# YuePanEdward/GH-ICP

Measured on AMD Instinct MI355X. Metric: registered_pairs_per_sec, higher is better.
Workload: dtype f64

## Files before the change

gh-icp_amd/csrc/bsc.hip:

```cpp
#include "frontend.h"
#include "devmath.h"
#include "bsc_dev.h"

namespace {

__global__ __launch_bounds__(BT) void k_bsc(GridArgs G, const int* __restrict__ kp, BscConst C, uint8_t* __restrict__ feat, float* __restrict__ lcs) {
  gh_bsc_keypoint(G, C, (int)blockIdx.x, C.K, feat, lcs);
}

__global__ __launch_bounds__(256) void k_bsc_origins(const float* __restrict__ xyz, int stride, const int* __restrict__ kp, int K, float* __restrict__ lcs) {
  const int k = blockIdx.x * 256 + threadIdx.x;
  if (k >= K) return;
  const long long s = kp[k];
  lcs[(size_t)k * 12 + 9] = xyz[s * stride];
  lcs[(size_t)k * 12 + 10] = xyz[s * stride + 1];
  lcs[(size_t)k * 12 + 11] = xyz[s * stride + 2];
}

}

int gh_bsc_make_const(ghicp_ctx* ctx, float R, int dof, const int32_t* pattern_host, BscConst* out, float* r_search) {
  BscConst C;
  memset(&C, 0, sizeof(C));
  C.R = R;
  const double rs = std::sqrt(3.0) * (double)R;
  C.r2s = (float)(rs * rs);
  C.u = 2 * R / 7;
  const float delta = (float)(C.u * 0.5);
  C.den = 2 * delta * delta;
  C.r2c = (float)((1.5 * (double)C.u) * (1.5 * (double)C.u));
  C.area = (float)(M_PI * (double)R * (double)R);
  C.radius_w = std::sqrt(2.0) * (double)R;
  int ex = 0;
  (void)std::frexp((double)R * 0.5, &ex);
  C.dunit = std::ldexp(1.0, 24 - ex);
  C.dinv = std::ldexp(1.0, ex - 54);
  for (int i = 0; i < 7; i++) C.centre[i] = (float)((i + 0.5) * (double)C.u - (double)R);
  for (int i = 0; i < 98; i++) {
    C.pattern[i] = pattern_host[i];
    if (C.pattern[i] < 0 || C.pattern[i] > 48) return ctx->fail(GHICP_ERR_ARG, "BSC sample pattern entry %d out of [0,48]", i);
  }
  C.K = 0;
  C.nvar = (dof > 4) ? 4 : (dof > 0 ? 2 : 1);
  *out = C;
  *r_search = (float)rs;
  return GHICP_OK;
}

int gh_bsc_dev(ghicp_ctx* ctx, const float* xyz, long long m, int stride, const int32_t* kp, long long K, float R, int dof, const int32_t* pattern_host,
               uint8_t* feat, float* lcs) {
  if (K <= 0) return GHICP_OK;
  hipStream_t s = ctx->stream;
  BscConst C;
  float r_search_f = 0.f;
  GH_TRY(gh_bsc_make_const(ctx, R, dof, pattern_host, &C, &r_search_f));
  C.K = (int)K;
  DeviceGrid G;
  const GridSlots sl = {B_GRID2_KEYS, B_GRID2_KEYS2, B_GRID2_VALS, B_GRID2_VALS2, B_GRID2_START, B_GRID2_PTS};
  GH_TRY(gh_grid_build(ctx, xyz, m, stride, r_search_f * 1.0001f, sl, &G));
  GH_HIP(hipMemsetAsync(feat, 0, (size_t)4 * K * 56, s));
  hipLaunchKernelGGL(k_bsc_origins, dim3(cdiv(K, 256)), dim3(256), 0, s, xyz, stride, kp, (int)K, lcs);
  GridArgs A = {G.d, G.pts, G.start};
  hipEvent_t kt = ctx->kt_begin(KT_BSC);
  hipLaunchKernelGGL(k_bsc, dim3((unsigned)K), dim3(BT), 0, s, A, kp, C, feat, lcs);
  ctx->kt_end(KT_BSC, kt);
  GH_HIP(hipGetLastError());
  return GHICP_OK;
}

extern "C" int ghicp_bsc_encode(ghicp_ctx* ctx, const float* xyz, int64_t m, int stride, const int32_t* kp_idx, int64_t k, float radius, int dof,
                                const int32_t* pattern, uint8_t* feat, float* lcs) {
  GH_ENTER(ctx);
  GH_ARG(m >= 0 && m < (1ll << 31) - 2 && k >= 0 && k <= m && stride >= 3 && radius > 0.f && pattern != nullptr);
  Stager sg(ctx);
  const float* d;
  const int32_t* dk;
  uint8_t* df;
  float* dl;
  GH_TRY(sg.in_cloud(xyz, (size_t)m * stride, &d));
  GH_TRY(sg.in(kp_idx, (size_t)k, &dk));
  GH_TRY(sg.out(feat, (size_t)4 * k * 56, &df));
  GH_TRY(sg.out(lcs, (size_t)k * 12, &dl));
  GH_TRY(gh_bsc_dev(ctx, d, m, stride, dk, k, radius, dof, pattern, df, dl));
  return sg.finish();
}
```

gh-icp_amd/csrc/bsc_dev.h:

```cpp
#pragma once
#include "grid.h"
#include "devmath.h"
#include "bsc_exp_table.h"

struct BscConst {
  float R, r2s, u, den, r2c, area;
  double radius_w;
  double dunit, dinv;
  float centre[7];
  int pattern[98];
  int K, nvar;
};

constexpr int BT = 256;
constexpr int BSC_CAP = 2048;
constexpr int BSC_CHUNK = 512;

int gh_bsc_make_const(ghicp_ctx* ctx, float R, int dof, const int32_t* pattern_host, BscConst* out, float* r_search);

static __device__ const double gh_bsc_exp_tab[145] = {GH_BSC_EXP_TABLE};
__device__ inline float gh_bsc_expf(float xf, const double* __restrict__ tab) {
  const double x = (double)xf;
  int j = (int)(x * -32.0 + 0.5);
  j = j < 0 ? 0 : (j > 144 ? 144 : j);
  const double s = x + (double)j * 0.03125;
  double p = s * (1.0 / 720.0) + (1.0 / 120.0);
  p = s * p + (1.0 / 24.0);
  p = s * p + (1.0 / 6.0);
  p = s * p + 0.5;
  p = s * p + 1.0;
  p = s * p + 1.0;
  return (float)(tab[j] * p);
}

__device__ inline void gh_bsc_depth_add(unsigned long long* __restrict__ lo64, unsigned* __restrict__ carry, float depth, float ew, double dunit) {
  const unsigned d_off = (unsigned)((int)((double)depth * dunit) + (1 << 27));
  const unsigned w_int = (unsigned)((double)ew * 1073741824.0);
  const unsigned long long term = (unsigned long long)d_off * (unsigned long long)w_int;
  const unsigned long long old = atomicAdd(lo64, term);
  if (old + term < old) atomicAdd(carry, 1u);
}
__device__ inline double gh_bsc_depth_sum(unsigned long long lo64, unsigned carry, double pnum, double dinv) {
  const unsigned __int128 acc = ((unsigned __int128)carry << 64) | (unsigned __int128)lo64;
  const unsigned __int128 shift = (unsigned __int128)(unsigned long long)(pnum * 1073741824.0) << 27;
  const bool neg = acc < shift;
  const unsigned __int128 mag = neg ? shift - acc : acc - shift;
  const double d = (double)(unsigned long long)(mag >> 32) * 4294967296.0 + (double)(unsigned long long)(mag & 0xFFFFFFFFull);
  return (neg ? -d : d) * dinv;
}

__device__ inline int rearr_src(int type, int k) {
  switch (type) {
    case 1: return 48 - k;
    case 2: return (6 - k / 7) * 7 + k % 7;
    default: return (k / 7) * 7 + 6 - k % 7;
  }
}

__device__ inline void gh_bsc_keypoint(const GridArgs& G, const BscConst& C, int kk, int K, uint8_t* __restrict__ feat, float* __restrict__ lcs) {

  __shared__ double red[16];
  __shared__ double s_pnum[147], s_exp[145];
  __shared__ unsigned long long s_dlo[147];
  __shared__ unsigned s_dcarry[147];
  __shared__ float s_weight[147], s_depth[147];
  __shared__ float s_axes[9];
  __shared__ double s_stat[3][4];
  __shared__ unsigned s_bits[4][16];
  __shared__ float4 s_pts[BSC_CHUNK];
  __shared__ int s_scan[17];
  __shared__ float s_centre[8];
  const int tid = threadIdx.x;
  const float qx = lcs[(size_t)kk * 12 + 9], qy = lcs[(size_t)kk * 12 + 10], qz = lcs[(size_t)kk * 12 + 11];
  const int cx = gh_cell_coord(qx, G.d.mn[0], G.d.inv, G.d.dim[0]);
  const int cy = gh_cell_coord(qy, G.d.mn[1], G.d.inv, G.d.dim[1]);
  const int cz = gh_cell_coord(qz, G.d.mn[2], G.d.inv, G.d.dim[2]);

  double sx = 0, sy = 0, sz = 0, sw = 0;
  int cnt = 0;
  gh_for_runs(G.d, G.start, cx, cy, cz, [&](unsigned b, unsigned e) {
    for (unsigned q = b + tid; q < e; q += BT) {
      const float4 P = G.pts[q];
      const float dx = qx - P.x, dy = qy - P.y, dz = qz - P.z;
      float d2 = dx * dx;
      d2 += dy * dy;
      d2 += dz * dz;
      if (d2 < C.r2s) {
        cnt++;
        sx += (double)P.x; sy += (double)P.y; sz += (double)P.z;
        sw += C.radius_w - (double)sqrtf(d2);
      }
    }
  });
  sx = gh_block_sum(sx, red); sy = gh_block_sum(sy, red); sz = gh_block_sum(sz, red); sw = gh_block_sum(sw, red);
  int mm;
  const int my_base = gh_block_excl_scan(cnt, s_scan, &mm);
  const double mx = sx / (double)mm, my = sy / (double)mm, mz = sz / (double)mm;
  const bool packed = mm <= BSC_CAP;
  auto fill_chunk = [&](int c0) {
    int w = my_base;
    gh_for_runs(G.d, G.start, cx, cy, cz, [&](unsigned b, unsigned e) {
      for (unsigned q = b + tid; q < e; q += BT) {
        const float4 P = G.pts[q];
        const float dx = qx - P.x, dy = qy - P.y, dz = qz - P.z;
        float d2 = dx * dx;
        d2 += dy * dy;
        d2 += dz * dz;
        if (d2 < C.r2s) {
          if (w >= c0 && w < c0 + BSC_CHUNK) s_pts[w - c0] = make_float4(P.x, P.y, P.z, d2);
          w++;
        }
      }
    });
    __syncthreads();
  };

  double c00 = 0, c01 = 0, c02 = 0, c11 = 0, c12 = 0, c22 = 0;
  if (mm >= 3 && packed) {
    for (int c0 = 0; c0 < mm; c0 += BSC_CHUNK) {
      fill_chunk(c0);
      const int cn = min(BSC_CHUNK, mm - c0);
      for (int t = tid; t < cn; t += BT) {
        const float4 P = s_pts[t];
        const double w = (double)(float)(C.radius_w - (double)sqrtf(P.w));
        const double ex = (double)P.x - mx, ey = (double)P.y - my, ez = (double)P.z - mz;
        c00 += w * ex * ex; c01 += w * ex * ey; c02 += w * ex * ez;
        c11 += w * ey * ey; c12 += w * ey * ez; c22 += w * ez * ez;
      }
      __syncthreads();
    }
  } else if (mm >= 3) {
    gh_for_runs(G.d, G.start, cx, cy, cz, [&](unsigned b, unsigned e) {
      for (unsigned q = b + tid; q < e; q += BT) {
        const float4 P = G.pts[q];
        const float dx = qx - P.x, dy = qy - P.y, dz = qz - P.z;
        float d2 = dx * dx;
        d2 += dy * dy;
        d2 += dz * dz;
        if (d2 < C.r2s) {
          const double w = (double)(float)(C.radius_w - (double)sqrtf(d2));
          const double ex = (double)P.x - mx, ey = (double)P.y - my, ez = (double)P.z - mz;
          c00 += w * ex * ex; c01 += w * ex * ey; c02 += w * ex * ez;
          c11 += w * ey * ey; c12 += w * ey * ez; c22 += w * ez * ez;
        }
      }
    });
  }
  if (mm >= 3) {
    c00 = gh_block_sum(c00, red); c01 = gh_block_sum(c01, red); c02 = gh_block_sum(c02, red);
    c11 = gh_block_sum(c11, red); c12 = gh_block_sum(c12, red); c22 = gh_block_sum(c22, red);
  }
  if (tid == 0) {
    float X[3] = {1, 0, 0}, Y[3] = {0, 1, 0}, Z[3] = {0, 0, 1};
    if (mm >= 3) {
      const float da = (float)sw;
      double Cq[6] = {c00, c01, c02, c11, c12, c22};
      gh_quant_grid(Cq, 6);
      double a00 = (double)((float)Cq[0] / da), a01 = (double)((float)Cq[1] / da), a02 = (double)((float)Cq[2] / da),
             a11 = (double)((float)Cq[3] / da), a12 = (double)((float)Cq[4] / da), a22 = (double)((float)Cq[5] / da);
      double V[9];
      gh_jacobi3(a00, a01, a02, a11, a12, a22, V);
      const double ev[3] = {a00, a11, a22};
      int imax = 0, imin = 0;
      for (int i = 0; i < 3; i++) {
        if ((float)ev[i] > (float)ev[imax]) imax = i;
        if ((float)ev[i] < (float)ev[imin]) imin = i;
      }
      float P[3], N[3];
      for (int which = 0; which < 2; which++) {
        const int col = which == 0 ? imax : imin;
        const double e[3] = {V[0 * 3 + col], V[1 * 3 + col], V[2 * 3 + col]};
        int b = 0;
        if (fabs(e[1]) > fabs(e[b])) b = 1;
        if (fabs(e[2]) > fabs(e[b])) b = 2;
        const double sg = (e[b] < 0) ? -1.0 : 1.0;
        float* o = which == 0 ? P : N;
        for (int d = 0; d < 3; d++) o[d] = (float)(sg * e[d]);
      }
      const float M0 = P[1] * N[2] - P[2] * N[1], M1 = P[2] * N[0] - P[0] * N[2], M2 = P[0] * N[1] - P[1] * N[0];
      X[0] = P[0]; X[1] = P[1]; X[2] = P[2];
      Y[0] = M0; Y[1] = M1; Y[2] = M2;
      Z[0] = X[1] * Y[2] - X[2] * Y[1];
      Z[1] = X[2] * Y[0] - X[0] * Y[2];
      Z[2] = X[0] * Y[1] - X[1] * Y[0];
      const float nx = sqrtf((X[0] * X[0] + X[1] * X[1]) + X[2] * X[2]);
      const float ny = sqrtf((Y[0] * Y[0] + Y[1] * Y[1]) + Y[2] * Y[2]);
      for (int d = 0; d < 3; d++) { X[d] = X[d] / nx; Y[d] = Y[d] / ny; }
    }
    for (int d = 0; d < 3; d++) { s_axes[d] = X[d]; s_axes[3 + d] = Y[d]; s_axes[6 + d] = Z[d]; }
    float* o = &lcs[(size_t)kk * 12];
    for (int d = 0; d < 3; d++) { o[d] = X[d]; o[3 + d] = Y[d]; o[6 + d] = Z[d]; }
  }
  for (int i = tid; i < 147; i += BT) { s_pnum[i] = 0.0; s_dlo[i] = 0ull; s_dcarry[i] = 0u; }
  for (int i = tid; i < 145; i += BT) s_exp[i] = gh_bsc_exp_tab[i];
  if (tid < 7) s_centre[tid] = C.centre[tid];
  if (tid < 64) s_bits[tid >> 4][tid & 15] = 0u;
  __syncthreads();
  const float X0 = s_axes[0], X1 = s_axes[1], X2 = s_axes[2], Y0 = s_axes[3], Y1 = s_axes[4], Y2 = s_axes[5], Z0 = s_axes[6], Z1 = s_axes[7],
              Z2 = s_axes[8];

  auto splat = [&](float px, float py, float pz) {
    const float d0 = px - qx, d1 = py - qy, d2v = pz - qz;
    const float loc[3] = {(X0 * d0 + X1 * d1) + X2 * d2v, (Y0 * d0 + Y1 * d1) + Y2 * d2v, (Z0 * d0 + Z1 * d1) + Z2 * d2v};
#pragma unroll
    for (int pl = 0; pl < 3; pl++) {
      const float a = loc[pl == 2 ? 1 : 0], bb = loc[pl == 0 ? 1 : 2];
      const float depth = loc[pl == 0 ? 2 : (pl == 1 ? 1 : 0)] + C.R;
      for (int j = 0; j < 7; j++) {
        const float dy = bb - C.centre[j];
        const float dy2 = dy * dy;
        if (!(dy2 < C.r2c)) continue;
        for (int i = 0; i < 7; i++) {
          const float dx = a - C.centre[i];
          float dd = dx * dx;
          dd += dy2;
          if (dd < C.r2c) {
            const float ew = gh_bsc_expf(-dd / C.den, s_exp);
            atomicAdd(&s_pnum[i + 7 * j + 49 * pl], (double)ew);
            gh_bsc_depth_add(&s_dlo[i + 7 * j + 49 * pl], &s_dcarry[i + 7 * j + 49 * pl], depth, ew, C.dunit);
          }
        }
      }
    }
  };
  if (packed) {
    const int wave = tid >> 6, lane = tid & 63;
    const int sub = lane / 9, slot = lane % 9;
    const int di = slot % 3 - 1, dj = slot / 3 - 1;
    const float inv_u = 1.0f / C.u;
    for (int c0 = 0; c0 < mm; c0 += BSC_CHUNK) {
    fill_chunk(c0);
    const int cn = min(BSC_CHUNK, mm - c0);
    for (int t = tid; t < cn; t += BT) {
      const float4 P = s_pts[t];
      const float d0 = P.x - qx, d1 = P.y - qy, d2v = P.z - qz;
      s_pts[t] = make_float4((X0 * d0 + X1 * d1) + X2 * d2v, (Y0 * d0 + Y1 * d1) + Y2 * d2v, (Z0 * d0 + Z1 * d1) + Z2 * d2v, 0.f);
    }
    __syncthreads();
    const int nitem = cn * 3;
    for (int base = 0; base < nitem; base += 28) {
      const int w = base + wave * 7 + sub;
      if (lane < 63 && w < nitem) {
        const int t = w / 3, pl = w - 3 * t;
        const float4 L = s_pts[t];
        const float a = pl == 2 ? L.y : L.x, bb = pl == 0 ? L.y : L.z;
        const float depth = (pl == 0 ? L.z : (pl == 1 ? L.y : L.x)) + C.R;
        const float ta = (a + C.R) * inv_u, tb = (bb + C.R) * inv_u;
        const float fla = floorf(ta), flb = floorf(tb);
        const int bi = (int)fla, bj = (int)flb;
        auto cell = [&](int ci, int cj) {
          if (ci < 0 || ci >= 7 || cj < 0 || cj >= 7) return;
          const float dy = bb - s_centre[cj];
          const float dy2 = dy * dy;
          const float dx = a - s_centre[ci];
          float dd = dx * dx;
          dd += dy2;
          if (dy2 < C.r2c && dd < C.r2c) {
            const float ew = gh_bsc_expf(-dd / C.den, s_exp);
            atomicAdd(&s_pnum[ci + 7 * cj + 49 * pl], (double)ew);
            gh_bsc_depth_add(&s_dlo[ci + 7 * cj + 49 * pl], &s_dcarry[ci + 7 * cj + 49 * pl], depth, ew, C.dunit);
          }
        };
        cell(bi + di, bj + dj);
        const float fa = ta - fla, fb = tb - flb;
        if (fa < 1e-4f || fa > 0.9999f || fb < 1e-4f || fb > 0.9999f) {
          bool fx = false, fy = false;
          const int i2 = bi + 2 * di, j2 = bj + 2 * dj;
          if (di != 0 && i2 >= 0 && i2 < 7) { const float dx = a - s_centre[i2]; fx = dx * dx < C.r2c; }
          if (dj != 0 && j2 >= 0 && j2 < 7) { const float dy = bb - s_centre[j2]; fy = dy * dy < C.r2c; }
          if (fx) cell(i2, bj + dj);
          if (fy) cell(bi + di, j2);
          if (fx && fy) cell(i2, j2);
        }
      }
    }
    __syncthreads();
    }
  } else {
    gh_for_runs(G.d, G.start, cx, cy, cz, [&](unsigned b, unsigned e) {
      for (unsigned q = b + tid; q < e; q += BT) {
        const float4 P = G.pts[q];
        const float tx = qx - P.x, ty = qy - P.y, tz = qz - P.z;
        float d2 = tx * tx;
        d2 += ty * ty;
        d2 += tz * tz;
        if (!(d2 < C.r2s)) continue;
        splat(P.x, P.y, P.z);
      }
    });
  }
  __syncthreads();

  if (tid < 147) {
    const float ndens = (float)mm / C.area;
    float avg = (float)gh_bsc_depth_sum(s_dlo[tid], s_dcarry[tid], s_pnum[tid], C.dinv);
    avg = (s_pnum[tid] == 0.0) ? 0.0f : (float)((double)avg / s_pnum[tid]);
    const float garea = C.u * C.u;
    const float gdens = (float)(s_pnum[tid] / (double)garea);
    s_weight[tid] = (ndens != 0.0f) ? gdens / ndens : 0.0f;
    s_depth[tid] = avg;
  }
  __syncthreads();
  if (tid < 3) {
    const int off = 49 * tid;
    double avg_d = 0, var_d = 0, avg_w = 0, var_w = 0;
    for (int i = 0; i < 49; i++) {
      const int a = C.pattern[2 * i] + off, b = C.pattern[2 * i + 1] + off;
      avg_d += (double)(s_depth[a] - s_depth[b]);
      avg_w += (double)(s_weight[a] - s_weight[b]);
    }
    avg_d /= 49; avg_w /= 49;
    for (int i = 0; i < 49; i++) {
      const int a = C.pattern[2 * i] + off, b = C.pattern[2 * i + 1] + off;
      const double dd = (double)(s_depth[a] - s_depth[b]), dw = (double)(s_weight[a] - s_weight[b]);
      var_d += (dd - avg_d) * (dd - avg_d);
      var_w += (dw - avg_w) * (dw - avg_w);
    }
    var_d /= 49; var_w /= 49;
    s_stat[tid][0] = avg_d; s_stat[tid][1] = sqrt(var_d); s_stat[tid][2] = avg_w; s_stat[tid][3] = sqrt(var_w);
  }
  __syncthreads();
  for (int base = 0; base < 448; base += BT) {
    const int k = base + tid;
    for (int v = 0; v < C.nvar; v++) {
      bool bit = false;
      if (v == 0) {
        if (k < 147) bit = s_weight[k] > 0.1f;
        else if (k < 441) {
          const int r = k - 147, pl = r / 98, p = (r % 98) >> 1, off = 49 * pl;
          const int a = C.pattern[2 * p], b = C.pattern[2 * p + 1];
          if ((r & 1) == 0) {
            const double dd = (double)(s_depth[a + off] - s_depth[b + off]);
            bit = fabs(dd - s_stat[pl][0]) > s_stat[pl][1];
          } else if (!(s_weight[a] < 0.1f && s_weight[b] < 0.1f)) {
            const double dw = (double)(s_weight[a + off] - s_weight[b + off]);
            bit = fabs(dw - s_stat[pl][2]) > s_stat[pl][3];
          }
        }
      } else if (k >= 147 && k < 294) {
        static const int TR[4][3] = {{0, 0, 0}, {1, 2, 2}, {3, 2, 1}, {2, 1, 3}};
        const int r = k - 147, pl = r / 49, kk2 = r % 49;
        bit = s_weight[49 * pl + rearr_src(TR[v][pl], kk2)] > 0.1f;
      }
      const unsigned long long bal = __ballot(bit);
      if ((tid & 63) == 0 && k < 448) {
        s_bits[v][k >> 5] = (unsigned)bal;
        if (k + 32 < 448) s_bits[v][(k >> 5) + 1] = (unsigned)(bal >> 32);
      }
    }
  }
  __syncthreads();
  if (tid < 14 * C.nvar) {
    const int v = tid / 14, w = tid % 14;
    reinterpret_cast<unsigned*>(feat)[((size_t)v * K + kk) * 14 + w] = s_bits[v][w];
  }
}
```

Before: 441.9.

## Replace double weight atomics with integer sums and division with reciprocal refinement

Replaces the per-cell double-precision atomicAdd of Gaussian weights with a 64-bit integer weight sum built from the float's bit pattern, which also feeds the depth-offset computation. The division by den becomes a precomputed reciprocal with two FMA refinement steps, and the depth unit conversion moves from double to float. It also skips reloading the point chunk when all neighbours fit in one resident chunk. These changes aim to cut slow double atomics and double math in the hot splat loop, at the risk of small numeric differences in the weight and depth quantisation.

Result: no change. 444.6, median of 6 (+0.6%).

```diff
diff --git a/gh-icp_amd/csrc/bsc.hip b/gh-icp_amd/csrc/bsc.hip
--- a/gh-icp_amd/csrc/bsc.hip
+++ b/gh-icp_amd/csrc/bsc.hip
@@ -28,6 +28,7 @@
   C.u = 2 * R / 7;
   const float delta = (float)(C.u * 0.5);
   C.den = 2 * delta * delta;
+  gh_bsc_quot_const(C.den, &C.rden, &C.dd_min);
   C.r2c = (float)((1.5 * (double)C.u) * (1.5 * (double)C.u));
   C.area = (float)(M_PI * (double)R * (double)R);
   C.radius_w = std::sqrt(2.0) * (double)R;
diff --git a/gh-icp_amd/csrc/bsc_dev.h b/gh-icp_amd/csrc/bsc_dev.h
--- a/gh-icp_amd/csrc/bsc_dev.h
+++ b/gh-icp_amd/csrc/bsc_dev.h
@@ -2,9 +2,11 @@
 #include "grid.h"
 #include "devmath.h"
 #include "bsc_exp_table.h"
+#include "bsc_weight.h"
 
 struct BscConst {
   float R, r2s, u, den, r2c, area;
+  float rden, dd_min;
   double radius_w;
   double dunit, dinv;
   float centre[7];
@@ -33,16 +35,17 @@
   return (float)(tab[j] * p);
 }
 
-__device__ inline void gh_bsc_depth_add(unsigned long long* __restrict__ lo64, unsigned* __restrict__ carry, float depth, float ew, double dunit) {
-  const unsigned d_off = (unsigned)((int)((double)depth * dunit) + (1 << 27));
-  const unsigned w_int = (unsigned)((double)ew * 1073741824.0);
+__device__ inline unsigned gh_bsc_depth_units(float depth, float dunit) { return (unsigned)((int)(depth * dunit) + (1 << 27)); }
+__device__ inline void gh_bsc_cell_add(unsigned long long* __restrict__ wsum, unsigned long long* __restrict__ lo64, unsigned* __restrict__ carry, unsigned d_off, float ew) {
+  const unsigned w_int = gh_bsc_weight_int(ew);
+  atomicAdd(wsum, (unsigned long long)w_int);
   const unsigned long long term = (unsigned long long)d_off * (unsigned long long)w_int;
   const unsigned long long old = atomicAdd(lo64, term);
   if (old + term < old) atomicAdd(carry, 1u);
 }
-__device__ inline double gh_bsc_depth_sum(unsigned long long lo64, unsigned carry, double pnum, double dinv) {
+__device__ inline double gh_bsc_depth_sum(unsigned long long lo64, unsigned carry, unsigned long long wsum, double dinv) {
   const unsigned __int128 acc = ((unsigned __int128)carry << 64) | (unsigned __int128)lo64;
-  const unsigned __int128 shift = (unsigned __int128)(unsigned long long)(pnum * 1073741824.0) << 27;
+  const unsigned __int128 shift = (unsigned __int128)wsum << 27;
   const bool neg = acc < shift;
   const unsigned __int128 mag = neg ? shift - acc : acc - shift;
   const double d = (double)(unsigned long long)(mag >> 32) * 4294967296.0 + (double)(unsigned long long)(mag & 0xFFFFFFFFull);
@@ -60,8 +63,8 @@
 __device__ inline void gh_bsc_keypoint(const GridArgs& G, const BscConst& C, int kk, int K, uint8_t* __restrict__ feat, float* __restrict__ lcs) {
 
   __shared__ double red[16];
-  __shared__ double s_pnum[147], s_exp[145];
-  __shared__ unsigned long long s_dlo[147];
+  __shared__ double s_exp[145];
+  __shared__ unsigned long long s_wsum[147], s_dlo[147];
   __shared__ unsigned s_dcarry[147];
   __shared__ float s_weight[147], s_depth[147];
   __shared__ float s_axes[9];
@@ -191,11 +194,12 @@
     float* o = &lcs[(size_t)kk * 12];
     for (int d = 0; d < 3; d++) { o[d] = X[d]; o[3 + d] = Y[d]; o[6 + d] = Z[d]; }
   }
-  for (int i = tid; i < 147; i += BT) { s_pnum[i] = 0.0; s_dlo[i] = 0ull; s_dcarry[i] = 0u; }
+  for (int i = tid; i < 147; i += BT) { s_wsum[i] = 0ull; s_dlo[i] = 0ull; s_dcarry[i] = 0u; }
   for (int i = tid; i < 145; i += BT) s_exp[i] = gh_bsc_exp_tab[i];
   if (tid < 7) s_centre[tid] = C.centre[tid];
   if (tid < 64) s_bits[tid >> 4][tid & 15] = 0u;
   __syncthreads();
+  const float dunit = (float)C.dunit;
   const float X0 = s_axes[0], X1 = s_axes[1], X2 = s_axes[2], Y0 = s_axes[3], Y1 = s_axes[4], Y2 = s_axes[5], Z0 = s_axes[6], Z1 = s_axes[7],
               Z2 = s_axes[8];
 
@@ -205,7 +209,7 @@
 #pragma unroll
     for (int pl = 0; pl < 3; pl++) {
       const float a = loc[pl == 2 ? 1 : 0], bb = loc[pl == 0 ? 1 : 2];
-      const float depth = loc[pl == 0 ? 2 : (pl == 1 ? 1 : 0)] + C.R;
+      const unsigned d_off = gh_bsc_depth_units(loc[pl == 0 ? 2 : (pl == 1 ? 1 : 0)] + C.R, dunit);
       for (int j = 0; j < 7; j++) {
         const float dy = bb - C.centre[j];
         const float dy2 = dy * dy;
@@ -215,9 +219,8 @@
           float dd = dx * dx;
           dd += dy2;
           if (dd < C.r2c) {
-            const float ew = gh_bsc_expf(-dd / C.den, s_exp);
-            atomicAdd(&s_pnum[i + 7 * j + 49 * pl], (double)ew);
-            gh_bsc_depth_add(&s_dlo[i + 7 * j + 49 * pl], &s_dcarry[i + 7 * j + 49 * pl], depth, ew, C.dunit);
+            const float ew = gh_bsc_expf(gh_bsc_neg_quot(dd, C.den, C.rden, C.dd_min), s_exp);
+            gh_bsc_cell_add(&s_wsum[i + 7 * j + 49 * pl], &s_dlo[i + 7 * j + 49 * pl], &s_dcarry[i + 7 * j + 49 * pl], d_off, ew);
           }
         }
       }
@@ -228,8 +231,9 @@
     const int sub = lane / 9, slot = lane % 9;
     const int di = slot % 3 - 1, dj = slot / 3 - 1;
     const float inv_u = 1.0f / C.u;
+    const bool resident = mm >= 3 && mm <= BSC_CHUNK;
     for (int c0 = 0; c0 < mm; c0 += BSC_CHUNK) {
-    fill_chunk(c0);
+    if (!resident) fill_chunk(c0);
     const int cn = min(BSC_CHUNK, mm - c0);
     for (int t = tid; t < cn; t += BT) {
       const float4 P = s_pts[t];
@@ -244,7 +248,7 @@
         const int t = w / 3, pl = w - 3 * t;
         const float4 L = s_pts[t];
         const float a = pl == 2 ? L.y : L.x, bb = pl == 0 ? L.y : L.z;
-        const float depth = (pl == 0 ? L.z : (pl == 1 ? L.y : L.x)) + C.R;
+        const unsigned d_off = gh_bsc_depth_units((pl == 0 ? L.z : (pl == 1 ? L.y : L.x)) + C.R, dunit);
         const float ta = (a + C.R) * inv_u, tb = (bb + C.R) * inv_u;
         const float fla = floorf(ta), flb = floorf(tb);
         const int bi = (int)fla, bj = (int)flb;
@@ -256,9 +260,8 @@
           float dd = dx * dx;
           dd += dy2;
           if (dy2 < C.r2c && dd < C.r2c) {
-            const float ew = gh_bsc_expf(-dd / C.den, s_exp);
-            atomicAdd(&s_pnum[ci + 7 * cj + 49 * pl], (double)ew);
-            gh_bsc_depth_add(&s_dlo[ci + 7 * cj + 49 * pl], &s_dcarry[ci + 7 * cj + 49 * pl], depth, ew, C.dunit);
+            const float ew = gh_bsc_expf(gh_bsc_neg_quot(dd, C.den, C.rden, C.dd_min), s_exp);
+            gh_bsc_cell_add(&s_wsum[ci + 7 * cj + 49 * pl], &s_dlo[ci + 7 * cj + 49 * pl], &s_dcarry[ci + 7 * cj + 49 * pl], d_off, ew);
           }
         };
         cell(bi + di, bj + dj);
@@ -293,10 +296,12 @@
 
   if (tid < 147) {
     const float ndens = (float)mm / C.area;
-    float avg = (float)gh_bsc_depth_sum(s_dlo[tid], s_dcarry[tid], s_pnum[tid], C.dinv);
-    avg = (s_pnum[tid] == 0.0) ? 0.0f : (float)((double)avg / s_pnum[tid]);
+    const unsigned long long wsum = s_wsum[tid];
+    const double pnum = (double)wsum * (1.0 / 1073741824.0);
+    float avg = (float)gh_bsc_depth_sum(s_dlo[tid], s_dcarry[tid], wsum, C.dinv);
+    avg = (wsum == 0ull) ? 0.0f : (float)((double)avg / pnum);
     const float garea = C.u * C.u;
-    const float gdens = (float)(s_pnum[tid] / (double)garea);
+    const float gdens = (float)(pnum / (double)garea);
     s_weight[tid] = (ndens != 0.0f) ? gdens / ndens : 0.0f;
     s_depth[tid] = avg;
   }
diff --git a/gh-icp_amd/csrc/bsc_weight.h b/gh-icp_amd/csrc/bsc_weight.h
--- /dev/null
+++ b/gh-icp_amd/csrc/bsc_weight.h
@@ -0,0 +1,29 @@
+#pragma once
+#include <cstdint>
+#include <cstring>
+
+#if defined(__HIPCC__)
+#define GH_BSC_FN __host__ __device__ inline
+#else
+#define GH_BSC_FN inline
+#endif
+
+GH_BSC_FN float gh_bsc_neg_quot(float dd, float den, float rden, float dd_min) {
+  const float n = -dd;
+  if (!(dd >= dd_min)) return n / den;
+  const float q0 = n * rden;
+  const float q1 = __builtin_fmaf(__builtin_fmaf(-den, q0, n), rden, q0);
+  return __builtin_fmaf(__builtin_fmaf(-den, q1, n), rden, q1);
+}
+inline void gh_bsc_quot_const(float den, float* rden, float* dd_min) {
+  const bool tame = den >= 0x1p-20f && den <= 0x1p20f;
+  *rden = tame ? 1.0f / den : 0.0f;
+  *dd_min = tame ? 0x1p-100f : __builtin_inff();
+}
+
+GH_BSC_FN unsigned gh_bsc_weight_int(float ew) {
+  unsigned b;
+  memcpy(&b, &ew, 4);
+  const unsigned m = (b & 0x007FFFFFu) | 0x00800000u;
+  return m << ((b >> 23) - 120u);
+}
```
